# wischmcj/pyQSM

Measured on AMD Instinct MI355X. Metric: Mpoints/s DBSCAN (1M-pt synthetic forest, eps=0.1, min_neighbors=10), higher is better.
Workload: dtype f64; 1 GPU; 1000000-point synthetic tree cloud (configs[1]), DBSCAN eps=0.1 min_neighbors=10, 20 clusters; replicas at N>1; points_per_gpu=1000000, parallelism=replicas x1

## Files before the change

### pyqsm_amd/csrc/dbscan.hip

```cpp
#include "grid.hpp"

#include <atomic>
#include <cfloat>
#include <chrono>
#include <cmath>
#include <optional>
#include <type_traits>
#include <vector>

namespace pyqsm {

static constexpr int kNoRoot = 0x7FFFFFFF;

__device__ __forceinline__ double sqdist(double ax, double ay, double az, double bx, double by,
                                         double bz) {
  double t0 = ax - bx, t1 = ay - by, t2 = az - bz;
  double d = t0 * t0;
  d = d + t1 * t1;
  d = d + t2 * t2;
  return d;
}


#define FOR_STENCIL(c, st, dir, q, body)                           \
// ... 73 lines not shown
  if (two) s_in[i + 1] = a.y, s_hi[i + 1] = b.y;
}

static constexpr int kStragglers = 6;
static constexpr int kMaxChunks = 3;
static constexpr int kRestSegs = 64;
__device__ constexpr int kRunOrder[9] = {4, 3, 5, 1, 7, 0, 2, 6, 8};

__device__ __forceinline__ void stencil_bounds(int c, Stencil st, const CellDir& dir, int (&qb)[9], int (&qe)[9]) {
  int cells[18], q[18];
#pragma unroll
  for (int r = 0; r < 9; ++r) {
    const int row = c + (kRunOrder[r] % 3 - 1) * st.nx + (kRunOrder[r] / 3 - 1) * st.nxy;
    cells[2 * r] = row - 1;
    cells[2 * r + 1] = row + 2;
  }
  dir.begins(cells, q);
#pragma unroll
  for (int r = 0; r < 9; ++r) {
    qb[r] = q[2 * r];
    qe[r] = q[2 * r + 1];
  }
}

template <class CO, bool F32>
__global__ __launch_bounds__(256) void k_core_tiled(int n, const GridPlan* __restrict__ plan,
                                                    const DirWord* __restrict__ dwords,
                                                    const int32_t* __restrict__ dslots,
                                                    const int32_t* __restrict__ cell_of, CO co, double r2,
                                                    float neg_k, float ramp_a, float ramp_b ,
                                                    int min_pts, uint8_t* __restrict__ core,
                                                    int32_t* __restrict__ rest,
                                                    int32_t* __restrict__ rest_cnt , int seg_cap,
                                                    int* __restrict__ parent, int* __restrict__ min_orig,
                                                    uint32_t* __restrict__ bits ,
                                                    int32_t* __restrict__ seam , int seam_cap,
                                                    int max_chunks,
                                                    unsigned long long* __restrict__ tests ,
    unsigned long long* __restrict__ st ) {
  __shared__ TileLds L;
  __shared__ TileLdsF32 LF;
  stamped(st, [&] {
  const CellDir dir{dwords, dslots};
  const int lane = threadIdx.x & 63, w = __builtin_amdgcn_readfirstlane(threadIdx.x >> 6);
  const int p0 = (blockIdx.x * 4 + w) * 64;
  if (p0 >= n || !plan->ok) return;
  const Stencil st = plan_stencil(plan);
  const int ncell = plan->ncell;
  const int p = p0 + lane;
  const bool live = p < n;
  double x = 0.0, y = 0.0, z = 0.0;
  float fx = 0.0f, fy = 0.0f, fz = 0.0f;
  if constexpr (F32) {
    if (live) {
      const float4 v = co.p[p];
      fx = v.x, fy = v.y, fz = v.z;
    }
  } else {
    if (live) co.get(p, x, y, z);
  }
  const Tile t = wave_tile(p0, n, st, ncell, dir, cell_of);
  int cnt = 0;
  float2v acc_in = {0.0f, 0.0f}, acc_hi = {0.0f, 0.0f};
  const float fmin_pts = float(min_pts);
  bool deferred = false;
  int chunks = 0;
  int staged = 0;
  int band = 0;
  const auto hand_on = [&](unsigned long long und) {
// ... 76 lines not shown
          }
          for (; j < m; j += 2)
            pair(*reinterpret_cast<const float2v*>(&LF.x[w][j]), *reinterpret_cast<const float2v*>(&LF.y[w][j]),
                 *reinterpret_cast<const float2v*>(&LF.z[w][j]));
        } else {
          if (q < t.qe[r]) co.get(q, L.x[w][lane], L.y[w][lane], L.z[w][lane]);
          __builtin_amdgcn_wave_barrier();
#pragma unroll 4
          for (int j = 0; j < m; ++j)
            cnt += sqdist(x, y, z, L.x[w][j], L.y[w][j], L.z[w][j]) <= r2;
        }
        staged += m;
        __builtin_amdgcn_wave_barrier();
        const unsigned long long und =
            F32 ? __ballot(live && acc_in.x + acc_in.y < fmin_pts) : __ballot(live && cnt < min_pts);
        ++chunks;
        if ((__popcll(und) <= kStragglers || chunks >= max_chunks) &&
            !(ri == 8 && base + 64 >= t.qe[r])) {
          hand_on(und);
          break;
        }
      }
    }
    if constexpr (F32) {
      if (!deferred)
        hand_on(__ballot(live && acc_in.x + acc_in.y < fmin_pts && acc_hi.x + acc_hi.y >= fmin_pts));
    }
  }
  if (live && cnt >= 0) {
    const bool is_core = ramped ? acc_in.x + acc_in.y >= fmin_pts : cnt >= min_pts;
    core[p] = is_core;
    co.mark_core(p, is_core);
  }
  if (live) {
    parent[p] = p;
    min_orig[p] = 0x7F7F7F7F;
    if (p <= n / 32) bits[p] = 0u;
    if (p == 0) bits[n / 32 + 1] = 0u;
    for (int i = p; i < seam_cap; i += n) seam[i] = 0;
  }
  if (tests && lane == 0) {
    atomicAdd(tests + (blockIdx.x & 255), static_cast<unsigned long long>(staged));
    if (band) atomicAdd(tests + 256 + (blockIdx.x & 255), static_cast<unsigned long long>(band));
  }
  });
}

struct Runs9 {
  int qb[9];
  int pre[10];
  __device__ __forceinline__ int at(int g) const {
    int q = qb[0] + g;
#pragma unroll
    for (int r = 1; r < 9; ++r) q = g >= pre[r] ? qb[r] + (g - pre[r]) : q;
    return q;
  }
};
static constexpr int kRunBatch = 3;
__device__ __forceinline__ int lane_bound(bool act, int c, int j, Stencil st, const CellDir& dir) {
  const int r = int((0x862071534ull >> (4 * (j >> 1))) & 15ull);
  const int cell = c + (r % 3 - 1) * st.nx + (r / 3 - 1) * st.nxy + ((j & 1) ? 2 : -1);
  int b = 0;
  if (act) {
    const DirWord w = dir.words[cell >> 5];
    b = dir.slots[CellDir::slot_of(w, cell)];
  }
  return b;
}
__device__ __forceinline__ Runs9 runs_of_lanes(int bound, int k) {
  Runs9 t;
  t.pre[0] = 0;
#pragma unroll
  for (int r = 0; r < 9; ++r) {
// ... 85 lines not shown
      cur = next;
    }
  }
  return cur;
}

__device__ __forceinline__ void unite(int* parent, int a, int b) {
  int ra = find_root(parent, a), rb = find_root(parent, b);
  while (ra != rb) {
    if (link_prio(ra) < link_prio(rb)) {
      int t = ra;
      ra = rb;
      rb = t;
    }
    const int old = atomicCAS(parent + ra, ra, rb);
    if (old == ra) break;
    ra = find_root(parent, old);
    rb = find_root(parent, rb);
  }
}


__global__ __launch_bounds__(1024) void k_sub_rep(int n, const int32_t* __restrict__ sub_of,
                                                 const uint8_t* __restrict__ core,
                                                 const int32_t* __restrict__ order,
                                                 int* __restrict__ parent,
                                                 const int32_t* __restrict__ cell_of,
                                                 int4* __restrict__ rec,
                                                 int* __restrict__ run_min,
                                                 int4* __restrict__ list,
                                                 int32_t* __restrict__ list_cnt, const GridPlan* __restrict__ plan,
                                                 int4* __restrict__ list_xyz,
                                                 const DirWord* __restrict__ dwords,
    unsigned long long* __restrict__ st ) {
  stamped(st, [&] {
  if (!plan->ok) return;
  const int nx = plan->nx, ny = plan->ny;
  const int lane = threadIdx.x & 63, w = threadIdx.x >> 6;
  const int base = blockIdx.x * 1024 + w * 64;
  const int p = base + lane;
  const bool live = p < n;
  int sid = 0, s = n, e = n, ord = 0x7FFFFFFF, cell = 0;
  bool c = false;
  const bool c_prev = base >= 64 && p - 64 < n && core[p - 64];
  const bool c_next = p + 64 < n && core[p + 64];
  const int o_next = c_next ? order[p + 64] : 0x7FFFFFFF;
  if (live) {
    sid = sub_of[p];
    c = core[p];
    if (c) ord = order[p];
    cell = cell_of[p];
    const int2 run = *reinterpret_cast<const int2*>(rec + sid);
    s = run.x;
    e = run.x + run.y;
  }
  const unsigned long long cb = __ballot(c);
  int lead = -1;
  const int s0 = __shfl(s, 0, 64);
  if (s0 < base && s0 >= base - 64) {
    const unsigned long long f = __ballot(c_prev && base - 64 + lane >= s0);
    if (f) lead = base - 64 + __ffsll(f) - 1;
  } else {
    for (int q0 = s0; q0 < base; q0 += 64) {
      const int q = q0 + lane;
      const unsigned long long f = __ballot(q < base && core[q]);
      if (f) {
        lead = q0 + __ffsll(f) - 1;
        break;
      }
    }
  }
  int rep = -1;
  if (c) {
    if (s < base && lead >= 0) {
      rep = lead;
    } else {
      const int lo = s > base ? s - base : 0;
      rep = base + __ffsll(cb & (~0ull << lo)) - 1;
    }
    parent[p] = rep;
  }
  const bool is_rep = c && rep == p;
  int mn = ord;
  const int seg_end = e - base < 64 ? e - base : 64;
#pragma unroll
  for (int off = 1; off < 64; off <<= 1) {
    const int o = __shfl_down(mn, off, 64);
    if (lane + off < seg_end) mn = o < mn ? o : mn;
  }
  const unsigned long long tail = __ballot(is_rep && e > base + 64);
  if (tail) {
    const int t = __ffsll(tail) - 1;
    const int et = __shfl(e, t, 64);
    int m2 = base + 64 + lane < et ? o_next : 0x7FFFFFFF;
    for (int q = base + 128 + lane; q < et; q += 64)
      if (core[q]) m2 = min(m2, order[q]);
#pragma unroll
    for (int off = 32; off > 0; off >>= 1) {
      const int o = __shfl_xor(m2, off, 64);
      m2 = o < m2 ? o : m2;
    }
    if (lane == t) mn = min(mn, m2);
  }
  if (is_rep) {
    rec[sid].z = rep;
    run_min[rep] = mn;
  }
  __shared__ int wcount[16], wbase[16];
  const unsigned long long b = __ballot(is_rep);
  if (lane == 0) wcount[w] = __popcll(b);
  __syncthreads();
  if (threadIdx.x == 0) {
    int tot = 0;
    for (int k = 0; k < 16; ++k) tot += wcount[k];
    int base2 = tot ? atomicAdd(list_cnt, tot) : 0;
    for (int k = 0; k < 16; ++k) {
      wbase[k] = base2;
      base2 += wcount[k];
    }
  }
  __syncthreads();
  if (is_rep) {
    const int slot = wbase[w] + __popcll(b & ((1ull << lane) - 1ull));
    const int c1 = cell;
    list[slot] = make_int4(rep, c1, CellDir::slot_of(dwords[c1 >> 5], c1), e - rep);
    list_xyz[slot] = make_int4(c1 % nx, (c1 / nx) % ny, c1 / (nx * ny), sid & 7);
  }
  });
}

__constant__ signed char kSubOffsets[62][3] = {{1,0,0}, {-1,1,0}, {0,1,0}, {1,1,0}, {-1,-1,1}, {0,-1,1}, {1,-1,1}, {-1,0,1}, {0,0,1}, {1,0,1}, {-1,1,1}, {0,1,1}, {1,1,1}, {2,0,0}, {-2,1,0}, {2,1,0}, {-2,2,0}, {-1,2,0}, {0,2,0}, {1,2,0}, {2,2,0}, {-2,-2,1}, {-1,-2,1}, {0,-2,1}, {1,-2,1}, {2,-2,1}, {-2,-1,1}, {2,-1,1}, {-2,0,1}, {2,0,1}, {-2,1,1}, {2,1,1}, {-2,2,1}, {-1,2,1}, {0,2,1}, {1,2,1}, {2,2,1}, {-2,-2,2}, {-1,-2,2}, {0,-2,2}, {1,-2,2}, {2,-2,2}, {-2,-1,2}, {-1,-1,2}, {0,-1,2}, {1,-1,2}, {2,-1,2}, {-2,0,2}, {-1,0,2}, {0,0,2}, {1,0,2}, {2,0,2}, {-2,1,2}, {-1,1,2}, {0,1,2}, {1,1,2}, {2,1,2}, {-2,2,2}, {-1,2,2}, {0,2,2}, {1,2,2}, {2,2,2}};

template <int kThreads>
__device__ __forceinline__ void block_append(bool take, int value, int32_t* __restrict__ list,
                                             int32_t* __restrict__ cnt) {
  constexpr int kWaves = kThreads / 64;
  __shared__ int wcount[kWaves], wbase[kWaves];
  const unsigned long long b = __ballot(take);
  const int lane = threadIdx.x & 63, w = threadIdx.x >> 6;
  if (lane == 0) wcount[w] = __popcll(b);
  __syncthreads();
  if (threadIdx.x == 0) {
    int tot = 0;
    for (int k = 0; k < kWaves; ++k) tot += wcount[k];
    int base = tot ? atomicAdd(cnt, tot) : 0;
    for (int k = 0; k < kWaves; ++k) {
      wbase[k] = base;
      base += wcount[k];
    }
  }
  __syncthreads();
  if (take) list[wbase[w] + __popcll(b & ((1ull << lane) - 1ull))] = value;
}

static constexpr int kFlagsThreads = 256, kFlagsPer = 16, kFlagsPerBlock = kFlagsThreads * kFlagsPer;
__device__ __forceinline__ void flags_role(int b, int n, const uint8_t* __restrict__ core,
                                           int32_t* __restrict__ rest, int32_t* __restrict__ rest_cnt) {
  constexpr int kWaves = kFlagsThreads / 64;
  __shared__ int fcount[kWaves], fbase[kWaves];
// ... 73 lines not shown
  const int before = __shfl_up(r, 1, 64);
  const bool many = __popcll(__ballot(lane == 0 || before != r)) > kFoldRuns;
  if (many && active && v < vmin[r]) atomicMin(min_orig + r, v);
  const int fold = many ? 0x7FFFFFFF : wave_fold_by_root(active, r, v);
  const bool has = fold != 0x7FFFFFFF;
  const unsigned long long hb = __ballot(has);
  int at = 0;
  if (lane == 0 && hb) at = atomicAdd(&f_cnt[grp], __popcll(hb));
  at = __shfl(at, 0, 64) + __popcll(hb & ((1ull << lane) - 1ull));
  if (has) {
    if (at < kFoldSlots) {
      f_root[grp][at] = r;
      f_min[grp][at] = fold;
    } else if (fold < vmin[r]) {
      atomicMin(min_orig + r, fold);
    }
  }
  __syncthreads();
  if ((threadIdx.x & 255) < 64) {
    const bool mine = lane < min(f_cnt[grp], kFoldSlots);
    const int r1 = mine ? f_root[grp][lane] : -1;
    const int fold1 = wave_fold_by_root(mine, r1, mine ? f_min[grp][lane] : 0x7FFFFFFF);
    if (fold1 != 0x7FFFFFFF && fold1 < vmin[r1]) atomicMin(min_orig + r1, fold1);
  }
}

template <FlattenMode MODE>
__global__ __launch_bounds__(kFlagsThreads) void k_flatten_reps(const int4* __restrict__ list,
                                                      const int32_t* __restrict__ m_ptr,
                                                      int* parent, int max_steps ,
                                                      const int32_t* __restrict__ link2 ,
                                                      int32_t* __restrict__ seam ,
                                                      int32_t* __restrict__ pre, int32_t* __restrict__ pre_cnt,
                                                      int rep_blocks , int n,
                                                      const uint8_t* __restrict__ core,
                                                      int32_t* __restrict__ rest, int32_t* __restrict__ rest_cnt,
                                                      const GridPlan* __restrict__ plan) {
  constexpr int kThreads = kFlagsThreads;
  static_assert(kThreads == 256, "the list is cut in 256s");
  if constexpr (MODE == kFlattenLink || MODE == kFlattenRoots) {
    if (int(blockIdx.x) >= rep_blocks) {
      if (plan->ok) flags_role(blockIdx.x - rep_blocks, n, core, rest, rest_cnt);
      return;
    }
  }
  const int m = *m_ptr;
  const int s = blockIdx.x * kThreads + threadIdx.x;
  const bool active = s < m;
  if constexpr (MODE == kFlattenJump || MODE == kFlattenLink) {
    if (!active) return;
  }
  int p = -1, r = -1, slot = -1;
  if (active) {
    const int4 me = list[s];
    p = r = me.x;
    slot = me.z;
  }
  if constexpr (MODE == kFlattenJump) {
    int steps = 0;
    for (int nx = parent[r]; nx != r && steps < max_steps; nx = parent[r], ++steps) r = nx;
    if (r != p) parent[p] = r;
  } else if constexpr (MODE == kFlattenLink) {
    const int l = link2[s];
    int r2 = l >= 0 ? l : p;
    for (;;) {
      const int a = parent[r], b = parent[r2];
      if (a == r && b == r2) break;
      r = a;
      r2 = b;
    }
    if (r != p) parent[p] = r;
    if (r2 != r) unite(parent, r, r2);
  } else {
    if (active) {
      for (int nx = parent[r]; nx != r; nx = parent[r]) r = nx;
      if (r != p) parent[p] = r;
    }
    const int lane = threadIdx.x & 63;
    const int pc = __shfl_up(slot, 1, 64), pr = __shfl_up(r, 1, 64);
    const bool dup = lane != 0 && pc == slot && pr == r;
    if (active && !dup) {
      int* const word = seam + slot;
      const int old = atomicCAS(word, 0, r + 1);
      if (old != 0 && old != r + 1 && old != -1) *word = -1;
    }
    block_append<kThreads>(active && r == p, p, pre, pre_cnt);
  }
}

static constexpr int kSubPerWave = 4;

struct SubNbr {
  int q0, n2, rep;
};
__device__ __forceinline__ SubNbr sub_neighbour(bool active, const int4 at, int dx, int dy, int dz, int nx, int ny,
                                                const CellDir& dir, const int4* __restrict__ rec) {
  const int gx = 2 * (at.x - 1) + (at.w & 1) - dx, gy = 2 * (at.y - 1) + ((at.w >> 1) & 1) - dy,
            gz = 2 * (at.z - 1) + ((at.w >> 2) & 1) - dz;
  const int c2 = (((gz >> 1) + 1) * ny + ((gy >> 1) + 1)) * nx + ((gx >> 1) + 1);
  const int oct = (gx & 1) | ((gy & 1) << 1) | ((gz & 1) << 2);
  SubNbr out{0, 0, -1};
  DirWord w{0u, 0u};
  if (active) w = dir.words[c2 >> 5];
  if ((w.bits >> (c2 & 31)) & 1u) {
    const int b2 = dir.slots[CellDir::slot_of(w, c2)];
    const int4 r = rec[b2 * 8 + oct];
    if (r.y > 0) {
      out.q0 = r.x;
      out.n2 = r.y;
      out.rep = r.z;
    }
  }
  return out;
}

template <class CO, bool LINK2>
__global__ __launch_bounds__(256) void k_hook_sub(const int4* __restrict__ list,
                                                  const int4* __restrict__ list_xyz,
// ... 169 lines not shown
#pragma unroll
      for (int l = 0; l < 2; ++l)
        if ((dw[l].bits >> ((c2 - l * layer) & 31)) & 1u) word[l] = seam[CellDir::slot_of(dw[l], c2 - l * layer)];
      const int own = __shfl(word[0], g9 * 9 + 4, 64);
      const unsigned long long bad = __ballot(
          act && (own == -1 || (word[0] != 0 && word[0] != own) || (word[1] != 0 && word[1] != own)));
#pragma unroll
      for (int g = 0; g < 7; ++g) {
        if ((bad >> (9 * g)) & 0x1FFull) seam_leaders |= rem & (~rem + 1ull);
        rem &= rem - 1;
      }
    }
    if (seam_leaders) {
      const int leader = 63 - __clzll(leaders & (~0ull >> (63 - k)));
      const bool take = live && ((seam_leaders >> leader) & 1ull);
      const unsigned long long todo = __ballot(take);
      int at = 0;
      if (k == 0) at = atomicAdd(&todo_cnt, __popcll(todo));
      at = __shfl(at, 0, 64);
      if (take) todo_list[at + __popcll(todo & ((1ull << k) - 1ull))] = s0 + k;
    }
    __syncthreads();
    const int cnt = todo_cnt;
    if (seam_cnt && threadIdx.x == 0 && cnt) atomicAdd(seam_cnt, static_cast<unsigned long long>(cnt));
    for (int i = wv; i < cnt; i += kSeamThreads / 64) {
      const int s = __builtin_amdgcn_readfirstlane(todo_list[i]);
      seam_unite(list[s], list_xyz[s], k, o_dx, o_dy, o_dz, nx, ny, dir, rec, co, r2, core, parent);
    }
    __syncthreads();
  }
  });
}

template <class CO>
__global__ __launch_bounds__(256) void k_union_points(int n, Stencil st,
                                                      const DirWord* __restrict__ dwords,
                                                      const int32_t* __restrict__ dslots,
                                                      const int32_t* __restrict__ cell_of, CO co, double r2,
                                                      const uint8_t* __restrict__ core, int* parent) {
  const CellDir dir{dwords, dslots};
  int p = blockIdx.x * 256 + threadIdx.x;
  if (p >= n || !core[p]) return;
  double x, y, z;
  co.get(p, x, y, z);
  const int c = cell_of[p];
  const volatile int* vparent = parent;
  int rp = find_root(parent, p);
  FOR_STENCIL(c, st, dir, q, {
    if (q < p && core[q] && co.d2(q, x, y, z) <= r2) {
      if (vparent[q] != rp) {
        unite(parent, p, q);
        rp = find_root(parent, p);
      }
    }
  })
}

__global__ __launch_bounds__(256) void k_flatten(int n, const uint8_t* __restrict__ core,
                                                 int* __restrict__ parent, const GridPlan* __restrict__ plan) {
  int p = blockIdx.x * 256 + threadIdx.x;
  if (!plan->ok || p >= n || !core[p]) return;
  int r = p;
  for (int nx = parent[r]; nx != r; nx = parent[r]) r = nx;
  parent[p] = r;
}

// ... 194 lines not shown
    for (int k = 0; k < kRunBatch; ++k) {
      if (i0 + k >= m) break;
      const Runs9 t = runs_of_lanes(bound, k);
      const int pk = __builtin_amdgcn_readlane(p, 18 * k);
      const double xk = __shfl(x, 18 * k, 64), yk = __shfl(y, 18 * k, 64), zk = __shfl(z, 18 * k, 64);
      int best = kNoRoot;
      for (int g0 = 0; g0 < t.pre[9]; g0 += 64) {
        const int g = g0 + lane;
        if (g < t.pre[9]) {
          const int q = t.at(g);
          if (core[q] && co.d2(q, xk, yk, zk) <= r2) {
            const int mo = min_orig[parent[parent[parent[q]]]];
            best = mo < best ? mo : best;
          }
        }
      }
#pragma unroll
      for (int off = 32; off > 0; off >>= 1) {
        const int o = __shfl_xor(best, off, 64);
        best = o < best ? o : best;
      }
      if (lane == 0)
        labels[order[pk]] = best == kNoRoot ? int64_t(-1) : int64_t(cluster_number(best, n_roots, bits, wpre));
    }
  }
  });
}

static double dbscan_r2(double eps, bool radius_inclusive) {
  return radius_inclusive ? eps * eps : nextafter(eps * eps, 0.0);
}

static int cluster_binned(Ctx* c, int64_t n, double eps, int32_t min_pts, bool radius_inclusive, const DevGrid& g,
                          const SubCells& sub, const GridPlan* d_plan, int64_t* labels, uint8_t* is_core,
                          const int32_t** count_out) {
  const bool fine = g.cell <= eps * (1.0 + 1.0 / 524288.0);
  const int N = int(n);
  const dim3 grid(ceil_div(n, 256)), block(256);
  const Stencil st{g.nx, g.nx * g.ny};
  const CellDir dir = cell_dir(g);
  const double r2 = dbscan_r2(eps, radius_inclusive);
  uint8_t* core;
  int *parent, *min_orig;
  uint32_t* bits;
  PQ_TRY(c->arena.get(size_t(n), &core));
  PQ_TRY(c->arena.get(size_t(n), &parent));
  PQ_TRY(c->arena.get(size_t(n), &min_orig));
  PQ_TRY(c->arena.get(size_t(n / 32) + 2, &bits));
  int32_t* const pre_cnt = reinterpret_cast<int32_t*>(bits + n / 32 + 1);
  const size_t seam_cap = fine ? size_t(n) + size_t(g.start ? g.ncell >> 5 : g.ncell >> 12) + 3 : 0;
  int32_t *seam, *pre;
  PQ_TRY(c->arena.get(seam_cap, &seam));
  PQ_TRY(c->arena.get(size_t(n), &pre));
  if (fine && g.start) PQ_HIP(hipMemsetAsync(seam, 0, seam_cap * 4, c->stream));
  int32_t *roots, *wpre;
  PQ_TRY(c->arena.get(size_t(n), &roots));
  PQ_TRY(c->arena.get(size_t(n / 32) + 1, &wpre));
  int4* list;
  int32_t* list_cnt;
  int* run_min;
  PQ_TRY(c->arena.get(size_t(n), &run_min));
  PQ_TRY(c->arena.get(size_t(n), &list));
  int4* list_xyz;
  PQ_TRY(c->arena.get(size_t(n), &list_xyz));
  int32_t* link2;
  PQ_TRY(c->arena.get(size_t(n), &link2));
  list_cnt = sub.zeroed4;
  int32_t* const roots_cnt = list_cnt + 1;
  int32_t* rest;
  const int core_blocks = int(ceil_div(n, 256));
  const int seg_cap = ceil_div(core_blocks, kRestSegs) * 256;
  PQ_TRY(c->arena.get(std::max<size_t>(size_t(n), size_t(seg_cap) * kRestSegs), &rest));
  int32_t* const rest_segs = list_cnt + 4;
  {
    StampScope ps(c, "dbscan_core");
    unsigned long long* d_tests = nullptr;
    if (c->prof >= 2) {
      PQ_TRY(c->arena.get(512, &d_tests));
      PQ_HIP(hipMemsetAsync(d_tests, 0, 512 * 8, c->stream));
    }
    const int max_chunks = std::min(32, std::max(kMaxChunks, (kMaxChunks * min_pts + 9) / 10));
    {
      const StampKernel pk(c, "k_core_tiled", grid.x);
      const CoreRamp cr = core_ramp(r2);
      const bool f32 = cr.usable(min_pts);
      on_coords(g, [&](auto co) {
        const auto launch = [&](auto kernel) {
          hipLaunchKernelGGL(kernel, grid, block, 0, c->stream, N, d_plan, dir.words, dir.slots, g.cell_of, co, r2, -cr.K,
                             cr.A, cr.B, min_pts, core, rest, rest_segs, seg_cap, parent, min_orig, bits, seam,
                             g.start ? 0 : int(seam_cap), max_chunks, d_tests, pk.slots);
        };
        if constexpr (std::is_same_v<decltype(co), CoordsF32>) {
          if (f32) return launch(k_core_tiled<CoordsF32, true>);
        }
        launch(k_core_tiled<decltype(co), false>);
      });
    }
    if (d_tests) {
      unsigned long long h[512];
      PQ_TRY(fetch(c, h, d_tests, 512));
      unsigned long long tot = 0, band = 0;
      for (int i = 0; i < 256; ++i) tot += h[i], band += h[256 + i];
      c->timers["core_pair_tests"].launches += int64_t(tot) * 64;
      c->timers["core_band_lanes"].launches += int64_t(band);
    }
    const dim3 gr(std::min<int64_t>(8192, ceil_div(n, 64)));
    unsigned long long* const st_rest = stamp_slots(c, gr.x);
    on_coords(g, [&](auto co) {
      hipLaunchKernelGGL(k_core_rest<decltype(co)>, gr, block, 0, c->stream, rest, rest_segs, seg_cap, d_plan, dir.words, dir.slots,
                         g.cell_of, co, r2, min_pts, core, st_rest);
    });
    PQ_HIP(hipGetLastError());
    if (getenv("PYQSM_DBSCAN_TRACE")) {
      int32_t h[kRestSegs];
      PQ_TRY(fetch(c, h, rest_segs, kRestSegs));
      long long tot = 0;
      for (int32_t v : h) tot += v;
      fprintf(stderr, "core pass: %lld stragglers\n", tot);
    }
  }
  {
    StampScope ps(c, "dbscan_union");
    const dim3 gf(ceil_div(n, kFlagsPerBlock));
    if (fine) {
      hipLaunchKernelGGL(k_sub_rep, dim3(ceil_div(n, 1024)), dim3(1024), 0, c->stream, N, sub.sub_of, core,
                         g.order, parent, g.cell_of, sub.rec, run_min, list, list_cnt, d_plan, list_xyz, dir.words,
                         stamp_slots(c, ceil_div(n, 1024)));
      {
        static const bool use_link2 = [] {
          const char* e = getenv("PYQSM_DBSCAN_LINK2");
          return e ? atoi(e) != 0 : true;
        }();
        int per_cu[2] = {use_link2 ? 8 : 16, 32};
        if (const char* e_cu = getenv("PYQSM_UNION_BLOCKS_PER_CU")) {
          per_cu[0] = per_cu[1] = atoi(e_cu);
          if (const char* comma = strchr(e_cu, ',')) per_cu[1] = atoi(comma + 1);
        }
        const int64_t full = ceil_div(n, 4 * kSubPerWave), full_u = ceil_div(n, kSeamThreads);
        const int64_t cu_u = std::max(1, per_cu[1] * 256 / kSeamThreads);
        const dim3 gh(per_cu[0] > 0 ? std::min<int64_t>(full, int64_t(c->cu_count) * per_cu[0]) : full),
            gu(per_cu[1] > 0 ? std::min<int64_t>(full_u, int64_t(c->cu_count) * cu_u) : full_u);
        const bool trace = getenv("PYQSM_DBSCAN_TRACE") != nullptr;
        {
          const StampKernel pk(c, "k_hook_sub", gh.x);
          on_coords(g, [&](auto co) {
            if (use_link2)
              hipLaunchKernelGGL((k_hook_sub<decltype(co), true>), gh, block, 0, c->stream, list, list_xyz, list_cnt,
                                 d_plan, dir.words, dir.slots, sub.rec, co, r2, core, parent, link2, pk.slots);
            else
              hipLaunchKernelGGL((k_hook_sub<decltype(co), false>), gh, block, 0, c->stream, list, list_xyz, list_cnt,
                                 d_plan, dir.words, dir.slots, sub.rec, co, r2, core, parent, link2, pk.slots);
          });
        }
        int32_t tm = 0;
        std::vector<int32_t> hp, root_of;
        std::vector<int4> hl;
        const auto snapshot = [&](std::vector<int64_t>* hist) -> int {
          PQ_TRY(fetch(c, &tm, list_cnt));
          hp.assign(static_cast<size_t>(n), 0);
          hl.assign(static_cast<size_t>(tm), make_int4(0, 0, 0, 0));
// ... 13 lines not shown
        };
        const auto count_roots = [&] {
          int64_t roots = 0;
          for (int32_t s2 = 0; s2 < tm; ++s2) roots += root_of[size_t(hl[size_t(s2)].x)] == hl[size_t(s2)].x;
          return roots;
        };
        int64_t links = 0, crossing = 0;
        if (trace) {
          std::vector<int64_t> hist(66, 0);
          PQ_TRY(snapshot(&hist));
          fprintf(stderr, "hook pass: %d sub-cells, %lld roots; chain depth histogram:", tm, (long long)count_roots());
          for (int d = 0; d < 66; ++d)
            if (hist[size_t(d)]) fprintf(stderr, " %d:%lld", d, (long long)hist[size_t(d)]);
          fprintf(stderr, "\n");
          if (use_link2) {
            std::vector<int32_t> h2(static_cast<size_t>(tm), -1);
            PQ_HIP(hipMemcpy(h2.data(), link2, size_t(tm) * 4, hipMemcpyDeviceToHost));
            for (int32_t s2 = 0; s2 < tm; ++s2) {
              if (h2[size_t(s2)] < 0) continue;
              ++links;
              crossing += root_of[size_t(h2[size_t(s2)])] != root_of[size_t(hl[size_t(s2)].x)];
            }
          }
        }
        static const int jump = [] {
          const char* e = getenv("PYQSM_FLATTEN_JUMP");
          return e ? atoi(e) : 12;
        }();
        const auto flatten = [&](auto mode, int max_steps, bool host_flags) {
          constexpr int threads = kFlagsThreads;
          const int rep_blocks = int(ceil_div(n, threads));
          hipLaunchKernelGGL(k_flatten_reps<decltype(mode)::value>, dim3(rep_blocks + (host_flags ? gf.x : 0)),
                             dim3(threads), 0, c->stream, list, list_cnt, parent, max_steps, link2, seam,
                             pre, pre_cnt, rep_blocks, N, core, rest, list_cnt + 3, d_plan);
        };
        if (jump > 0) flatten(std::integral_constant<FlattenMode, kFlattenJump>{}, jump, false);
        if (use_link2) {
          flatten(std::integral_constant<FlattenMode, kFlattenLink>{}, 0, true);
          if (trace) {
            PQ_TRY(snapshot(nullptr));
            fprintf(stderr, "link pass: %lld recorded, %lld crossed trees, %lld roots left\n", (long long)links,
                    (long long)crossing, (long long)count_roots());
          }
          flatten(std::integral_constant<FlattenMode, kFlattenWords>{}, 0, false);
        } else {
          flatten(std::integral_constant<FlattenMode, kFlattenRoots>{}, 0, true);
        }
        unsigned long long* d_seams = nullptr;
        if (trace) {
          PQ_TRY(c->arena.get(1, &d_seams));
          PQ_HIP(hipMemsetAsync(d_seams, 0, 8, c->stream));
        }
        {
          const int fold_blocks = int(ceil_div(n, kSeamThreads));
          const StampKernel pk(c, "k_union_sub", gu.x + fold_blocks);
          on_coords(g, [&](auto co) {
            hipLaunchKernelGGL(k_union_sub<decltype(co)>, dim3(gu.x + fold_blocks), dim3(kSeamThreads), 0, c->stream, list,
                               list_xyz, list_cnt, d_plan, dir.words, dir.slots, seam, sub.rec, co, r2, core, parent,
                               int(gu.x), run_min, min_orig, d_seams, pk.slots);
          });
        }
        if (trace) {
          unsigned long long h = 0;
          PQ_TRY(fetch(c, &h, d_seams));
          fprintf(stderr, "seam union: %llu sub-cells took the 62-offset path\n", h);
        }
        const dim3 gp(std::min<int64_t>(ceil_div(n, kFoldThreads), int64_t(c->cu_count) * 8));
        hipLaunchKernelGGL(k_fold_roots, gp, dim3(kFoldThreads), 0, c->stream, pre, pre_cnt, parent, min_orig, roots,
                           roots_cnt, d_plan);
      }
      PQ_HIP(hipGetLastError());
    } else {
      PQ_TRY(stamp_mark(c));
      on_coords(g, [&](auto co) {
        hipLaunchKernelGGL(k_union_points<decltype(co)>, grid, block, 0, c->stream, N, st, dir.words, dir.slots, g.cell_of, co,
                           r2, core, parent);
      });
      hipLaunchKernelGGL(k_flatten, grid, block, 0, c->stream, N, core, parent, d_plan);
      hipLaunchKernelGGL(k_point_min, grid, block, 0, c->stream, N, core, parent, g.order, min_orig, roots,
                         roots_cnt, d_plan);
      hipLaunchKernelGGL(k_noncore_list, gf, dim3(kFlagsThreads), 0, c->stream, N, core, rest,
                         list_cnt + 3, d_plan);
    }
    const dim3 gn(std::min<int64_t>(ceil_div(n, kNumberThreads), c->cu_count));
    hipLaunchKernelGGL(k_number, gn, dim3(kNumberThreads), 0, c->stream, N, roots, roots_cnt, min_orig, bits, wpre,
                       list_cnt + 2, d_plan, stamp_slots(c, gn.x));
    PQ_HIP(hipGetLastError());
  }
  {
    StampScope ps(c, "dbscan_label");
    const dim3 gb(ceil_div(n, kLabelThreads));
    unsigned long long* const st_labels = stamp_slots(c, gb.x);
    on_coords(g, [&](auto co) {
      hipLaunchKernelGGL(k_labels<decltype(co)>, gb, dim3(kLabelThreads), 0, c->stream, N, rest, list_cnt + 3, d_plan,
                         dir.words, dir.slots, g.cell_of, co, r2, core, parent, min_orig, roots_cnt, bits, wpre, g.order, labels,
                         is_core, st_labels);
    });
    PQ_HIP(hipGetLastError());
    if (getenv("PYQSM_DBSCAN_TRACE")) {
      int32_t h = 0;
      PQ_TRY(fetch(c, &h, list_cnt + 3));
      fprintf(stderr, "label pass: %d non-core points listed\n", h);
    }
  }
  *count_out = roots_cnt;
  return 0;
// ... 22 lines not shown
};
static int dbscan_device(Ctx* c, const double* xyz, int64_t n, double eps, int32_t min_pts,
                         bool radius_inclusive, int64_t* labels, uint8_t* is_core, int64_t* n_clusters,
                         DirReadout* readout = nullptr) {
  if (!(eps > 0) || !std::isfinite(eps)) return fail(PYQSM_EINVAL, "eps must be positive");
  if (n == 0) {
    if (n_clusters) *n_clusters = 0;
    return 0;
  }
  const double cell = eps * (1.0 + 1.0 / 1048576.0);
  const int64_t max_cells = int64_t(1) << 28;
  if (!c->plan_pinned) {
    PQ_HIP(hipHostMalloc(&c->plan_pinned, 2 * sizeof(GridPlan), hipHostMallocMapped | hipHostMallocCoherent));
    memset(c->plan_pinned, 0, 2 * sizeof(GridPlan));
  }
  GridPlan* const h_plan = static_cast<GridPlan*>(c->plan_pinned);
  GridPlan* h_plan_dev;
  PQ_HIP(hipHostGetDevicePointer(reinterpret_cast<void**>(&h_plan_dev), c->plan_pinned, 0));
  if (++c->plan_seq == 0) c->plan_seq = 1;
  const unsigned seq = c->plan_seq;
  GridPlan* d_plan;
  int32_t* zeroed;
  PQ_TRY(c->arena.get(2, &d_plan));
  PQ_TRY(c->arena.get(size_t(octant_zeroed_ints()), &zeroed));
  const char* plan_env = getenv("PYQSM_DBSCAN_PLAN");
  const char* bin_env = getenv("PYQSM_DBSCAN_BIN");
  const char* f32_env = getenv("PYQSM_COORD_F32");
  const bool speculate = c->plan_hint.valid && !(plan_env && !strcmp(plan_env, "host")) && !bin_env &&
                         !(f32_env && !strcmp(f32_env, "0")) && n <= (int64_t(1) << 25);
  const PlanHint hint = speculate ? c->plan_hint : PlanHint{};
  DevGrid g;
  SubCells sub;
  const int32_t* count = nullptr;
  std::optional<StampScope> bin_scope(std::in_place, c, "dbscan_bin");
  PlanRecords rec{};
  PQ_TRY(plan_grid_device(c, xyz, n, cell, max_cells, hint, d_plan, h_plan_dev, seq, zeroed, octant_zeroed_ints(),
                          speculate ? &rec : nullptr));
  const Arena::Mark mark = c->arena.mark();
  if (speculate) {
    PQ_TRY(bin_octants_planned(c, xyz, n, cell, hint, rec, d_plan, zeroed, &g, &sub));
    bin_scope.reset();
    if (!readout)
      PQ_TRY(cluster_binned(c, n, eps, min_pts, radius_inclusive, g, sub, d_plan, labels, is_core, &count));
  }
  PQ_TRY(wait_plan(c, h_plan, seq));
  const bool hit = speculate && h_plan[0].ok;
  if (!hit) {
    c->arena.rewind(mark);
    PlanHint next;
    if (!bin_scope) bin_scope.emplace(c, "dbscan_bin");
    PQ_TRY(stamp_mark(c));
    PQ_TRY(bin_octants_host(c, xyz, n, cell, max_cells, h_plan[0], zeroed, &h_plan[1], d_plan + 1, &g, &sub, &next));
    PQ_TRY(stamp_mark(c));
    bin_scope.reset();
    if (next.valid) c->plan_hint = next;
    if (!readout)
      PQ_TRY(cluster_binned(c, n, eps, min_pts, radius_inclusive, g, sub, d_plan + 1, labels, is_core, &count));
  }
  if (c->prof >= 1) {
    c->timers["dbscan_f32_records"].launches += g.p4 ? 1 : 0;
    c->timers[hit ? "dbscan_plan_hit" : "dbscan_plan_miss"].launches += 1;
  }
  if (readout) {
    const GridPlan& pl = hit ? h_plan[0] : h_plan[1];
    readout->dims[0] = pl.nx;
    readout->dims[1] = pl.ny;
    readout->dims[2] = pl.nz;
    const int64_t entries = int64_t(pl.ncell) + 1;
    if (entries > readout->cap)
      return fail(PYQSM_ERANGE, "octant directory: %lld entries, room for %lld", (long long)entries,
                  (long long)readout->cap);
    int32_t* d_begin;
    PQ_TRY(c->arena.get(size_t(entries), &d_begin));
    read_directory(c, g, pl.ncell, d_begin);
    PQ_HIP(hipGetLastError());
    PQ_TRY(fetch(c, readout->begin_host, d_begin, size_t(entries)));
    return 0;
  }
  if (n_clusters) {
    int32_t h = 0;
    PQ_TRY(fetch(c, &h, count));
    *n_clusters = h;
  }
  return 0;
}

}

using namespace pyqsm;

// ... 99 lines not shown
```

### pyqsm_amd/csrc/grid.hip

```cpp
#include "grid.hpp"

#include "block_scan.hpp"

#include <atomic>
#include <cmath>
#include <type_traits>

namespace pyqsm {

__device__ __forceinline__ unsigned long long ord_key(double x) {
  unsigned long long b = static_cast<unsigned long long>(__double_as_longlong(x));
  return (b >> 63) ? ~b : (b | 0x8000000000000000ull);
}
__host__ __device__ static inline double ord_val(unsigned long long k) {
  const unsigned long long b = (k >> 63) ? (k & 0x7FFFFFFFFFFFFFFFull) : ~k;
  double d;
  memcpy(&d, &b, 8);
  return d;
}

static constexpr int kBkMax = 16384;

struct BucketShape {
  int bits;
  int64_t nbk;
};
__host__ __device__ static inline BucketShape bucket_shape(int64_t ncell) {
  const int bits = ncell + 1 <= (int64_t(kBkMax) << 12) ? 12 : 13;
  return BucketShape{bits, (ncell + (int64_t(1) << bits)) >> bits};
}

__host__ __device__ static inline bool interior_slabs(const double* mn, const double* mx, double cell, double border,
                                                      int raw[3], double* tot) {
  bool ok = true;
  double t = 1.0;
  for (int a = 0; a < 3; ++a) {
    const double d = floor((mx[a] - mn[a]) / cell) + 1.0;
    if (!(d < 2.0e9)) ok = false;
    raw[a] = ok ? int(d) : 0;
    t *= d + border;
  }
  *tot = t;
  return ok;
}

static constexpr int kBoxVals = 7;
static int bbox_blocks(const Ctx* c, int64_t n) {
  return int(std::min<int64_t>(ceil_div(n, 256), int64_t(c->cu_count) * 2));
}
__global__ __launch_bounds__(256) void k_bbox(const double* __restrict__ xyz, int64_t n,
                                              unsigned long long* __restrict__ part ,
                                              int32_t* __restrict__ zero_buf, int zero_n,
    unsigned long long* __restrict__ st ) {
  __shared__ unsigned long long red[4][6];
  __shared__ int red_f32[4];
  stamped(st, [&] {
  unsigned long long mn[3] = {~0ull, ~0ull, ~0ull}, mx[3] = {0, 0, 0};
  bool f32ok = true;
  const int64_t stride = int64_t(gridDim.x) * blockDim.x;
  for (int64_t i = blockIdx.x * int64_t(blockDim.x) + threadIdx.x; i < n; i += stride) {
#pragma unroll
    for (int a = 0; a < 3; ++a) {
      const double v = xyz[3 * i + a];
      f32ok = f32ok && double(float(v)) == v;
      unsigned long long k = ord_key(v);
      mn[a] = k < mn[a] ? k : mn[a];
      mx[a] = k > mx[a] ? k : mx[a];
    }
  }
  for (int64_t q = blockIdx.x * int64_t(blockDim.x) + threadIdx.x; q < zero_n; q += stride) zero_buf[q] = 0;
  const bool wave_ok = __all(f32ok);
#pragma unroll
  for (int a = 0; a < 3; ++a) {
#pragma unroll
    for (int off = 32; off > 0; off >>= 1) {
      unsigned long long o1 = __shfl_down(mn[a], off, 64), o2 = __shfl_down(mx[a], off, 64);
      mn[a] = o1 < mn[a] ? o1 : mn[a];
      mx[a] = o2 > mx[a] ? o2 : mx[a];
    }
  }
  const int w = threadIdx.x >> 6;
  if ((threadIdx.x & 63) == 0) {
#pragma unroll
    for (int a = 0; a < 3; ++a) {
      red[w][a] = mn[a];
      red[w][3 + a] = mx[a];
    }
    red_f32[w] = wave_ok;
  }
  __syncthreads();
  if (threadIdx.x < 6) {
    unsigned long long v = red[0][threadIdx.x];
    for (int q = 1; q < 4; ++q) {
      const unsigned long long o = red[q][threadIdx.x];
      v = threadIdx.x < 3 ? (o < v ? o : v) : (o > v ? o : v);
    }
    part[size_t(blockIdx.x) * kBoxVals + threadIdx.x] = v;
  }
  if (threadIdx.x == 6)
    part[size_t(blockIdx.x) * kBoxVals + 6] = (red_f32[0] && red_f32[1] && red_f32[2] && red_f32[3]) ? 1ull : 0ull;
  });
}

// ... 214 lines not shown
    PQ_TRY(fetch(c, h, d_hist, 3 * kAxisBins));
    bool cut = false;
    for (int a = 0; a < 3; ++a) {
      const int32_t* ha = h + a * kAxisBins;
      int lo = 0, hi = kAxisBins - 1;
      int64_t acc = 0;
      while (lo < hi && acc + ha[lo] <= side) acc += ha[lo++];
      int64_t lost_a = acc;
      acc = 0;
      while (hi > lo && acc + ha[hi] <= side) acc += ha[hi--];
      lost_a += acc;
      if (hi - lo + 1 > (3 * kAxisBins) / 4 || !(inv[a] > 0)) continue;
      const double w = (box[3 + a] - box[a]) / double(kAxisBins);
      const double mn = box[a];
      box[a] = mn + w * double(lo);
      box[3 + a] = mn + w * double(hi + 1);
      lost_axis[a] = lost_a;
      cut = true;
    }
    if (!cut) break;
    *outside = (lost_axis[0] + lost_axis[1]) + lost_axis[2];
  }
  return 0;
}

int cloud_bbox(Ctx* c, const double* xyz, int64_t n, double mn[3], double mx[3], bool* all_f32,
               int32_t* zero_buf, int zero_n) {
  if (n <= 0) return fail(PYQSM_EINVAL, "bounding box of an empty cloud");
  const int blocks = bbox_blocks(c, n);
  unsigned long long *d_box = nullptr, *d_part = nullptr;
  PQ_TRY(c->arena.get(kBoxVals, &d_box));
  PQ_TRY(c->arena.get(size_t(blocks) * kBoxVals, &d_part));
  hipLaunchKernelGGL(k_bbox, dim3(blocks), dim3(256), 0, c->stream, xyz, n, d_part, zero_buf, zero_n,
                     static_cast<unsigned long long*>(nullptr));
  hipLaunchKernelGGL(k_bbox_fold, dim3(1), dim3(256), 0, c->stream, d_part, blocks, d_box, PlanIn{},
                     static_cast<GridPlan*>(nullptr));
  PQ_HIP(hipGetLastError());
  unsigned long long h_box[kBoxVals];
  PQ_TRY(fetch(c, h_box, d_box, kBoxVals));
  if (all_f32) *all_f32 = h_box[6] != 0;
  for (int a = 0; a < 3; ++a) {
    mn[a] = ord_val(h_box[a]);
    mx[a] = ord_val(h_box[3 + a]);
    if (!std::isfinite(mn[a]) || !std::isfinite(mx[a]))
      return fail(PYQSM_EINVAL, "point coordinates must be finite");
  }
  return 0;
}

static int build_grid_bucketed(Ctx* c, const double* xyz, int64_t n, DevGrid* g);
static bool bucketed_fits(const DevGrid& g);

int build_grid(Ctx* c, const double* xyz, int64_t n, double min_cell, int64_t max_cells,
               DevGrid* g, const double* bbox, bool f32_records) {
  if (n <= 0) return fail(PYQSM_EINVAL, "build_grid: empty cloud");
  if (n > 0x7FFFFF00LL) return fail(PYQSM_ERANGE, "more than 2^31 points per call");
  if (!(min_cell > 0) || !std::isfinite(min_cell))
    return fail(PYQSM_EINVAL, "cell edge must be positive and finite");
  double mn[3], mx[3];
  if (bbox) {
    for (int a = 0; a < 3; ++a) {
      mn[a] = bbox[a];
      mx[a] = bbox[3 + a];
    }
  } else {
    PQ_TRY(cloud_bbox(c, xyz, n, mn, mx));
  }
// ... 986 lines not shown
  ok = ok && tot <= double(in.max_cells);
  p.inv_cell = 1.0 / in.cell;
  p.rx = raw[0];
  p.ry = raw[1];
  p.rz = raw[2];
  p.nx = raw[0] + 2;
  p.ny = raw[1] + 2;
  p.nz = raw[2] + 2;
  const int64_t ncell = ok ? int64_t(p.nx) * p.ny * p.nz : 0;
  const BucketShape bs = bucket_shape(ncell);
  const int64_t nbk = bs.nbk;
  ok = ok && bs.bits == 12 && ncell <= in.hint.ncell && nbk <= in.hint.nbk &&
       (nbk <= kBkFusedScan) == (in.hint.fused != 0);
  p.ncell = ok ? int(ncell) : 0;
  p.nbk = ok ? int(nbk) : 0;
  p.bits = 12;
  p.ok = ok ? 1 : 0;
  p.seq = in.seq;
  return p;
}

__device__ void store_plan(GridPlan p, const PlanIn& in, GridPlan* __restrict__ plan) {
  *plan = p;
  if (in.host) {
    p.seq = 0;
    *in.host = p;
    __threadfence_system();
    *reinterpret_cast<volatile unsigned*>(&in.host->seq) = in.seq;
  }
}

int plan_grid_device(Ctx* c, const double* xyz, int64_t n, double cell, int64_t max_cells, const PlanHint& hint,
                     GridPlan* d_plan, GridPlan* h_plan, unsigned seq, int32_t* zero_buf, int zero_n,
                     PlanRecords* speculated) {
  if (n <= 0) return fail(PYQSM_EINVAL, "bounding box of an empty cloud");
  const int blocks = bbox_blocks(c, n);
  unsigned long long *d_box = nullptr, *d_part = nullptr;
  PQ_TRY(c->arena.get(kBoxVals, &d_box));
  PQ_TRY(c->arena.get(size_t(blocks) * kBoxVals, &d_part));
  hipLaunchKernelGGL(k_bbox, dim3(blocks), dim3(256), 0, c->stream, xyz, n, d_part, zero_buf, zero_n,
                     stamp_slots(c, blocks));
  if (speculated)
    *speculated = PlanRecords{d_part, blocks, max_cells, h_plan, seq};
  else
    hipLaunchKernelGGL(k_bbox_fold, dim3(1), dim3(256), 0, c->stream, d_part, blocks, d_box,
                       PlanIn{cell, max_cells, hint, h_plan, seq}, d_plan);
  PQ_HIP(hipGetLastError());
  return 0;
}

int octant_zeroed_ints() { return 2 * kBkMax + 5 + kZeroedExtra; }

static int enqueue_bucketed(Ctx* c, const double* xyz, int64_t n, const GridParams& gp, const int raw[3],
                            AxisMap am, bool mapped, int64_t nbk, int bits, bool f32,
                            int32_t* zeroed, const GridPlan* d_plan, DevGrid* g, SubCells* sub,
                            const PlanFold& pf = PlanFold{}) {
  int32_t *cell_tmp, *keyb, *rank_tmp, *bstart;
  uint32_t* word_tmp;
  int32_t *tot = zeroed, *cursor = zeroed + kBkMax;
  PointRec* keyed;
  void* bucketed;
  g->p4 = nullptr;
  g->sx = g->sy = g->sz = nullptr;
  g->start = nullptr;
  PQ_TRY(c->arena.get(size_t(nbk) << (bits - 5), &g->dir_words));
  PQ_TRY(c->arena.get(size_t(n) + size_t(nbk) + 1, &g->dir_slots));
  PQ_TRY(c->arena.get(size_t(n), &g->order));
  PQ_TRY(c->arena.get(size_t(n), &g->cell_of));
  if (f32) {
    float4* b4;
    PQ_TRY(c->arena.get(size_t(n), &g->p4));
    PQ_TRY(c->arena.get(size_t(n), &b4));
    bucketed = b4;
  } else {
// ... 458 lines not shown
```

### pyqsm_amd/csrc/grid.hpp

```cpp
#pragma once
#include "common.hpp"

namespace pyqsm {

struct alignas(8) DirWord {
  uint32_t bits, base;
};
struct CellDir {
  const DirWord* words;
  const int32_t* slots;
  __device__ __forceinline__ static int slot_of(const DirWord w, int c) {
    return int(w.base) + __popc(w.bits & ((1u << (c & 31)) - 1u));
  }
  __device__ __forceinline__ int begin(int c) const { return slots[slot_of(words[c >> 5], c)]; }
  template <int N>
  __device__ __forceinline__ void begins(const int (&c)[N], int (&out)[N]) const {
    DirWord w[N];
#pragma unroll
    for (int i = 0; i < N; ++i) w[i] = words[c[i] >> 5];
#pragma unroll
    for (int i = 0; i < N; ++i) out[i] = slots[slot_of(w[i], c[i])];
  }
};

// ... 229 lines not shown
    run += cnt;
  }
}
__device__ __forceinline__ void write_sub_records(int4* __restrict__ rec, int b, const int (&cnt)[8]) {
  write_sub_records_of(rec, b, [&](int o) { return cnt[o]; });
}
__device__ __forceinline__ void write_sub_records(int4* __restrict__ rec, int b, unsigned long long packed) {
  write_sub_records_of(rec, b, [&](int o) { return int((packed >> (8 * o)) & 255ull); });
}


struct GridPlan {
  double mn[3], mx[3];
  double inv_cell;
  int nx, ny, nz;
  int rx, ry, rz;
  int ncell;
  int nbk, bits;
  int all_f32;
  int ok;
  unsigned seq;
};
__device__ __forceinline__ Stencil plan_stencil(const GridPlan* p) { return Stencil{p->nx, p->nx * p->ny}; }

struct PlanRecords {
  const unsigned long long* part;
  int blocks;
  int64_t max_cells;
  GridPlan* h_plan;
  unsigned seq;
};
int plan_grid_device(Ctx* c, const double* xyz, int64_t n, double cell, int64_t max_cells, const PlanHint& hint,
                     GridPlan* d_plan, GridPlan* h_plan, unsigned seq, int32_t* zero_buf, int zero_n,
                     PlanRecords* speculated = nullptr);
int octant_zeroed_ints();
int bin_octants_planned(Ctx* c, const double* xyz, int64_t n, double cell, const PlanHint& hint,
                        const PlanRecords& rec, GridPlan* d_plan, int32_t* zeroed, DevGrid* g, SubCells* sub);
int bin_octants_host(Ctx* c, const double* xyz, int64_t n, double min_cell, int64_t max_cells, const GridPlan& box,
                     int32_t* zeroed, GridPlan* h_up, GridPlan* d_plan, DevGrid* g, SubCells* sub,
                     PlanHint* hint_out);

void read_directory(Ctx* c, const DevGrid& g, int64_t ncell, int32_t* begin_out);

int coarsen_grid(Ctx* c, const DevGrid& fine, int64_t n, int factor, DevGrid* coarse);

int ball_grid(Ctx* c, const double* d_src, int64_t n, double radius, DevGrid* g, double* cloud_box = nullptr);
int radius_grid(Ctx* c, const double* d_src, int64_t n, double radius, DevGrid* g);
int query_order(Ctx* c, const double* d_qry, int64_t m, const GridParams& rg, int64_t ncell, int32_t** perm);

int count_occupied(Ctx* c, const DevGrid& g, int64_t* occupied);

}
```

Baseline: 3900 Mpoints/s.

## Redistribute union-find init stores out of core kernel into later kernels

Removes the per-point initialisation of parent, min_orig, bits and seam from the core-counting kernel. The bits buffer is now zeroed inside the bbox kernel. Seam slots are cleared only at cell heads in k_sub_rep, and min_orig is set only for representatives in k_flatten_reps, with a separate init kernel for the coarse path. The aim is to cut dense global stores from the hot core kernel and write only the entries actually used, at the risk of leaving parent or seam entries uninitialised if a later stage reads slots the new sparse writes miss.

```diff
diff --git a/pyqsm_amd/csrc/dbscan.hip b/pyqsm_amd/csrc/dbscan.hip
--- a/pyqsm_amd/csrc/dbscan.hip
+++ b/pyqsm_amd/csrc/dbscan.hip
@@ -129,9 +129,6 @@
                                                     int min_pts, uint8_t* __restrict__ core,
                                                     int32_t* __restrict__ rest,
                                                     int32_t* __restrict__ rest_cnt , int seg_cap,
-                                                    int* __restrict__ parent, int* __restrict__ min_orig,
-                                                    uint32_t* __restrict__ bits ,
-                                                    int32_t* __restrict__ seam , int seam_cap,
                                                     int max_chunks,
                                                     unsigned long long* __restrict__ tests ,
     unsigned long long* __restrict__ st ) {
@@ -274,13 +271,6 @@
     core[p] = is_core;
     co.mark_core(p, is_core);
   }
-  if (live) {
-    parent[p] = p;
-    min_orig[p] = 0x7F7F7F7F;
-    if (p <= n / 32) bits[p] = 0u;
-    if (p == 0) bits[n / 32 + 1] = 0u;
-    for (int i = p; i < seam_cap; i += n) seam[i] = 0;
-  }
   if (tests && lane == 0) {
     atomicAdd(tests + (blockIdx.x & 255), static_cast<unsigned long long>(staged));
     if (band) atomicAdd(tests + 256 + (blockIdx.x & 255), static_cast<unsigned long long>(band));
@@ -432,6 +422,7 @@
                                                  int32_t* __restrict__ list_cnt, const GridPlan* __restrict__ plan,
                                                  int4* __restrict__ list_xyz,
                                                  const DirWord* __restrict__ dwords,
+                                                 int32_t* __restrict__ seam ,
     unsigned long long* __restrict__ st ) {
   stamped(st, [&] {
   if (!plan->ok) return;
@@ -445,6 +436,8 @@
   const bool c_prev = base >= 64 && p - 64 < n && core[p - 64];
   const bool c_next = p + 64 < n && core[p + 64];
   const int o_next = c_next ? order[p + 64] : 0x7FFFFFFF;
+  int c_before = -1;
+  if (lane == 0 && live && p > 0) c_before = cell_of[p - 1];
   if (live) {
     sid = sub_of[p];
     c = core[p];
@@ -454,6 +447,11 @@
     s = run.x;
     e = run.x + run.y;
   }
+  {
+    const int up = __shfl_up(cell, 1, 64);
+    if (lane != 0) c_before = up;
+  }
+  const bool head = live && cell != c_before;
   const unsigned long long cb = __ballot(c);
   int lead = -1;
   const int s0 = __shfl(s, 0, 64);
@@ -481,6 +479,9 @@
     parent[p] = rep;
   }
   const bool is_rep = c && rep == p;
+  int slot = 0;
+  if (head || is_rep) slot = CellDir::slot_of(dwords[cell >> 5], cell);
+  if (head && seam) seam[slot] = 0;
   int mn = ord;
   const int seg_end = e - base < 64 ? e - base : 64;
 #pragma unroll
@@ -521,10 +522,10 @@
   }
   __syncthreads();
   if (is_rep) {
-    const int slot = wbase[w] + __popcll(b & ((1ull << lane) - 1ull));
+    const int at = wbase[w] + __popcll(b & ((1ull << lane) - 1ull));
     const int c1 = cell;
-    list[slot] = make_int4(rep, c1, CellDir::slot_of(dwords[c1 >> 5], c1), e - rep);
-    list_xyz[slot] = make_int4(c1 % nx, (c1 / nx) % ny, c1 / (nx * ny), sid & 7);
+    list[at] = make_int4(rep, c1, slot, e - rep);
+    list_xyz[at] = make_int4(c1 % nx, (c1 / nx) % ny, c1 / (nx * ny), sid & 7);
   }
   });
 }
@@ -664,6 +665,7 @@
                                                       const int32_t* __restrict__ link2 ,
                                                       int32_t* __restrict__ seam ,
                                                       int32_t* __restrict__ pre, int32_t* __restrict__ pre_cnt,
+                                                      int* __restrict__ min_orig ,
                                                       int rep_blocks , int n,
                                                       const uint8_t* __restrict__ core,
                                                       int32_t* __restrict__ rest, int32_t* __restrict__ rest_cnt,
@@ -716,6 +718,7 @@
       const int old = atomicCAS(word, 0, r + 1);
       if (old != 0 && old != r + 1 && old != -1) *word = -1;
     }
+    if (active && r == p) min_orig[p] = 0x7F7F7F7F;
     block_append<kThreads>(active && r == p, p, pre, pre_cnt);
   }
 }
@@ -951,6 +954,13 @@
   });
 }
 
+__global__ __launch_bounds__(256) void k_init_points(int n, int* __restrict__ parent, int* __restrict__ min_orig) {
+  const int p = blockIdx.x * 256 + threadIdx.x;
+  if (p >= n) return;
+  parent[p] = p;
+  min_orig[p] = 0x7F7F7F7F;
+}
+
 template <class CO>
 __global__ __launch_bounds__(256) void k_union_points(int n, Stencil st,
                                                       const DirWord* __restrict__ dwords,
@@ -1211,8 +1221,8 @@
 }
 
 static int cluster_binned(Ctx* c, int64_t n, double eps, int32_t min_pts, bool radius_inclusive, const DevGrid& g,
-                          const SubCells& sub, const GridPlan* d_plan, int64_t* labels, uint8_t* is_core,
-                          const int32_t** count_out) {
+                          const SubCells& sub, const GridPlan* d_plan, uint32_t* bits, int64_t* labels,
+                          uint8_t* is_core, const int32_t** count_out) {
   const bool fine = g.cell <= eps * (1.0 + 1.0 / 524288.0);
   const int N = int(n);
   const dim3 grid(ceil_div(n, 256)), block(256);
@@ -1221,11 +1231,9 @@
   const double r2 = dbscan_r2(eps, radius_inclusive);
   uint8_t* core;
   int *parent, *min_orig;
-  uint32_t* bits;
   PQ_TRY(c->arena.get(size_t(n), &core));
   PQ_TRY(c->arena.get(size_t(n), &parent));
   PQ_TRY(c->arena.get(size_t(n), &min_orig));
-  PQ_TRY(c->arena.get(size_t(n / 32) + 2, &bits));
   int32_t* const pre_cnt = reinterpret_cast<int32_t*>(bits + n / 32 + 1);
   const size_t seam_cap = fine ? size_t(n) + size_t(g.start ? g.ncell >> 5 : g.ncell >> 12) + 3 : 0;
   int32_t *seam, *pre;
@@ -1266,8 +1274,7 @@
       on_coords(g, [&](auto co) {
         const auto launch = [&](auto kernel) {
           hipLaunchKernelGGL(kernel, grid, block, 0, c->stream, N, d_plan, dir.words, dir.slots, g.cell_of, co, r2, -cr.K,
-                             cr.A, cr.B, min_pts, core, rest, rest_segs, seg_cap, parent, min_orig, bits, seam,
-                             g.start ? 0 : int(seam_cap), max_chunks, d_tests, pk.slots);
+                             cr.A, cr.B, min_pts, core, rest, rest_segs, seg_cap, max_chunks, d_tests, pk.slots);
         };
         if constexpr (std::is_same_v<decltype(co), CoordsF32>) {
           if (f32) return launch(k_core_tiled<CoordsF32, true>);
@@ -1304,7 +1311,7 @@
     if (fine) {
       hipLaunchKernelGGL(k_sub_rep, dim3(ceil_div(n, 1024)), dim3(1024), 0, c->stream, N, sub.sub_of, core,
                          g.order, parent, g.cell_of, sub.rec, run_min, list, list_cnt, d_plan, list_xyz, dir.words,
-                         stamp_slots(c, ceil_div(n, 1024)));
+                         g.start ? nullptr : seam, stamp_slots(c, ceil_div(n, 1024)));
       {
         static const bool use_link2 = [] {
           const char* e = getenv("PYQSM_DBSCAN_LINK2");
@@ -1384,7 +1391,7 @@
           const int rep_blocks = int(ceil_div(n, threads));
           hipLaunchKernelGGL(k_flatten_reps<decltype(mode)::value>, dim3(rep_blocks + (host_flags ? gf.x : 0)),
                              dim3(threads), 0, c->stream, list, list_cnt, parent, max_steps, link2, seam,
-                             pre, pre_cnt, rep_blocks, N, core, rest, list_cnt + 3, d_plan);
+                             pre, pre_cnt, min_orig, rep_blocks, N, core, rest, list_cnt + 3, d_plan);
         };
         if (jump > 0) flatten(std::integral_constant<FlattenMode, kFlattenJump>{}, jump, false);
         if (use_link2) {
@@ -1424,6 +1431,7 @@
       PQ_HIP(hipGetLastError());
     } else {
       PQ_TRY(stamp_mark(c));
+      hipLaunchKernelGGL(k_init_points, grid, block, 0, c->stream, N, parent, min_orig);
       on_coords(g, [&](auto co) {
         hipLaunchKernelGGL(k_union_points<decltype(co)>, grid, block, 0, c->stream, N, st, dir.words, dir.slots, g.cell_of, co,
                            r2, core, parent);
@@ -1512,16 +1520,18 @@
   DevGrid g;
   SubCells sub;
   const int32_t* count = nullptr;
+  uint32_t* bits;
+  PQ_TRY(c->arena.get(size_t(n / 32) + 2, &bits));
   std::optional<StampScope> bin_scope(std::in_place, c, "dbscan_bin");
   PlanRecords rec{};
   PQ_TRY(plan_grid_device(c, xyz, n, cell, max_cells, hint, d_plan, h_plan_dev, seq, zeroed, octant_zeroed_ints(),
-                          speculate ? &rec : nullptr));
+                          reinterpret_cast<int32_t*>(bits), int(n / 32) + 2, speculate ? &rec : nullptr));
   const Arena::Mark mark = c->arena.mark();
   if (speculate) {
     PQ_TRY(bin_octants_planned(c, xyz, n, cell, hint, rec, d_plan, zeroed, &g, &sub));
     bin_scope.reset();
     if (!readout)
-      PQ_TRY(cluster_binned(c, n, eps, min_pts, radius_inclusive, g, sub, d_plan, labels, is_core, &count));
+      PQ_TRY(cluster_binned(c, n, eps, min_pts, radius_inclusive, g, sub, d_plan, bits, labels, is_core, &count));
   }
   PQ_TRY(wait_plan(c, h_plan, seq));
   const bool hit = speculate && h_plan[0].ok;
@@ -1535,7 +1545,7 @@
     bin_scope.reset();
     if (next.valid) c->plan_hint = next;
     if (!readout)
-      PQ_TRY(cluster_binned(c, n, eps, min_pts, radius_inclusive, g, sub, d_plan + 1, labels, is_core, &count));
+      PQ_TRY(cluster_binned(c, n, eps, min_pts, radius_inclusive, g, sub, d_plan + 1, bits, labels, is_core, &count));
   }
   if (c->prof >= 1) {
     c->timers["dbscan_f32_records"].launches += g.p4 ? 1 : 0;
diff --git a/pyqsm_amd/csrc/grid.hip b/pyqsm_amd/csrc/grid.hip
--- a/pyqsm_amd/csrc/grid.hip
+++ b/pyqsm_amd/csrc/grid.hip
@@ -51,6 +51,7 @@
 __global__ __launch_bounds__(256) void k_bbox(const double* __restrict__ xyz, int64_t n,
                                               unsigned long long* __restrict__ part ,
                                               int32_t* __restrict__ zero_buf, int zero_n,
+                                              int32_t* __restrict__ zero_buf2, int zero_n2,
     unsigned long long* __restrict__ st ) {
   __shared__ unsigned long long red[4][6];
   __shared__ int red_f32[4];
@@ -69,6 +70,7 @@
     }
   }
   for (int64_t q = blockIdx.x * int64_t(blockDim.x) + threadIdx.x; q < zero_n; q += stride) zero_buf[q] = 0;
+  for (int64_t q = blockIdx.x * int64_t(blockDim.x) + threadIdx.x; q < zero_n2; q += stride) zero_buf2[q] = 0;
   const bool wave_ok = __all(f32ok);
 #pragma unroll
   for (int a = 0; a < 3; ++a) {
@@ -349,7 +351,7 @@
   PQ_TRY(c->arena.get(kBoxVals, &d_box));
   PQ_TRY(c->arena.get(size_t(blocks) * kBoxVals, &d_part));
   hipLaunchKernelGGL(k_bbox, dim3(blocks), dim3(256), 0, c->stream, xyz, n, d_part, zero_buf, zero_n,
-                     static_cast<unsigned long long*>(nullptr));
+                     static_cast<int32_t*>(nullptr), 0, static_cast<unsigned long long*>(nullptr));
   hipLaunchKernelGGL(k_bbox_fold, dim3(1), dim3(256), 0, c->stream, d_part, blocks, d_box, PlanIn{},
                      static_cast<GridPlan*>(nullptr));
   PQ_HIP(hipGetLastError());
@@ -1402,14 +1404,14 @@
 
 int plan_grid_device(Ctx* c, const double* xyz, int64_t n, double cell, int64_t max_cells, const PlanHint& hint,
                      GridPlan* d_plan, GridPlan* h_plan, unsigned seq, int32_t* zero_buf, int zero_n,
-                     PlanRecords* speculated) {
+                     int32_t* zero_buf2, int zero_n2, PlanRecords* speculated) {
   if (n <= 0) return fail(PYQSM_EINVAL, "bounding box of an empty cloud");
   const int blocks = bbox_blocks(c, n);
   unsigned long long *d_box = nullptr, *d_part = nullptr;
   PQ_TRY(c->arena.get(kBoxVals, &d_box));
   PQ_TRY(c->arena.get(size_t(blocks) * kBoxVals, &d_part));
   hipLaunchKernelGGL(k_bbox, dim3(blocks), dim3(256), 0, c->stream, xyz, n, d_part, zero_buf, zero_n,
-                     stamp_slots(c, blocks));
+                     zero_buf2, zero_n2, stamp_slots(c, blocks));
   if (speculated)
     *speculated = PlanRecords{d_part, blocks, max_cells, h_plan, seq};
   else
diff --git a/pyqsm_amd/csrc/grid.hpp b/pyqsm_amd/csrc/grid.hpp
--- a/pyqsm_amd/csrc/grid.hpp
+++ b/pyqsm_amd/csrc/grid.hpp
@@ -285,7 +285,7 @@
 };
 int plan_grid_device(Ctx* c, const double* xyz, int64_t n, double cell, int64_t max_cells, const PlanHint& hint,
                      GridPlan* d_plan, GridPlan* h_plan, unsigned seq, int32_t* zero_buf, int zero_n,
-                     PlanRecords* speculated = nullptr);
+                     int32_t* zero_buf2, int zero_n2, PlanRecords* speculated = nullptr);
 int octant_zeroed_ints();
 int bin_octants_planned(Ctx* c, const double* xyz, int64_t n, double cell, const PlanHint& hint,
                         const PlanRecords& rec, GridPlan* d_plan, int32_t* zeroed, DevGrid* g, SubCells* sub);
```

Result: no change. 3905 Mpoints/s (median of 3 runs) (+0.1%).
